# KirillKryukov/naf

Measured on AMD Instinct MI355X. Metric: unnaf GB/s (uncompressed bases out) on 100 GB synthetic FASTA, higher is better.
Workload: dtype u8; 1 GPU; unnaf decode of a 100.0 GB synthetic-ACGT FASTA archive on one GPU (the size BASELINE.json's metric is quoted on; configs[1] at 10 GB rides along as cfg10_*), 100 records, 80-col lines; archive made in-run by the GPU ennaf; .naf 24739662224 B -> FASTA 99999995684 B, text + archive + decoded text resident in HBM; parallelism=one archive, one GPU, no data-path collective

## Files before the change

### naf_amd/csrc/emit.hip

```cpp
#include "ctx.h"
#include "wgscan.h"
#include "emit_core.h"
#include "packed.h"
#include <thread>

__device__ __forceinline__ void st_text16(u8 *p, const uint4 &v, int nt)
{
    if (nt) {
        u32x4 nv; nv.x = v.x; nv.y = v.y; nv.z = v.z; nv.w = v.w;
        __builtin_nontemporal_store(nv, (u32x4 *)p);
    } else *(uint4 *)p = v;
}

__global__ void k_len_flags(const u32 *units, u64 n, u64 *flag)
{
    u64 i = (u64)blockIdx.x * blockDim.x + threadIdx.x;
    if (i < n) flag[i] = units[i] != 0xFFFFFFFFu;
}
__global__ void k_len_acc(const u32 *units, u64 n, const u64 *ridx, u64 *rec_len, u64 N)
{
    u64 i = (u64)blockIdx.x * blockDim.x + threadIdx.x;
    if (i < n && ridx[i] < N) atomicAdd((unsigned long long *)&rec_len[ridx[i]], (unsigned long long)units[i]);
}

#define ZT_BYTES 16
#define ZT_TILE (256 * ZT_BYTES)
__device__ __forceinline__ u32 zero_byte_mask16(const u8 *p, u64 base, u64 n)
{
    u32 m = 0;
    if (base + ZT_BYTES <= n) {
        u64 a = ld64(p + base), b = ld64(p + base + 8);
#pragma unroll
        for (int i = 0; i < 8; i++) { if (((a >> (8 * i)) & 0xFF) == 0) m |= 1u << i; if (((b >> (8 * i)) & 0xFF) == 0) m |= 1u << (8 + i); }
    } else {
        for (int i = 0; i < ZT_BYTES; i++) if (base + i < n && p[base + i] == 0) m |= 1u << i;
    }
    return m;
}
__global__ __launch_bounds__(256) void k_zero_count(const u8 *p, u64 n, u64 *tile_cnt)
{
    __shared__ u64 lds[4];
    u64 base = (u64)blockIdx.x * ZT_TILE + (u64)threadIdx.x * ZT_BYTES;
    u64 c = base < n ? __popc(zero_byte_mask16(p, base, n)) : 0, tot;
    wg_scan_inclusive<u64, OpAdd>(c, &tot, lds);
    if (threadIdx.x == 0) tile_cnt[blockIdx.x] = tot;
}
__global__ __launch_bounds__(256) void k_zero_scatter(const u8 *p, u64 n, const u64 *tile_pre, u64 *pos_out, u64 cap)
{
    __shared__ u64 lds[4];
    u64 base = (u64)blockIdx.x * ZT_TILE + (u64)threadIdx.x * ZT_BYTES;
    u32 m = base < n ? zero_byte_mask16(p, base, n) : 0;
    u64 c = __popc(m), tot;
    u64 incl = wg_scan_inclusive<u64, OpAdd>(c, &tot, lds);
    u64 k = tile_pre[blockIdx.x] + incl - c;
    while (m) { int b = __ffs(m) - 1; m &= m - 1; if (k < cap) pos_out[k] = base + b; k++; }
}

#define MT_TILE (256 * 16)
__device__ __forceinline__ void mask_units16(const u8 *units, u64 base, u64 n, u32 w[4], u32 &sum, u32 &cnt)
{
    sum = 0; cnt = 0; w[0] = w[1] = w[2] = w[3] = 0xFFFFFFFFu;
    if (base >= n) return;
    const u64 a = ld64(units + base), b = ld64(units + base + 8);
    w[0] = (u32)a; w[1] = (u32)(a >> 32); w[2] = (u32)b; w[3] = (u32)(b >> 32);
    const u32 valid = n - base >= 16 ? 16u : (u32)(n - base);
#pragma unroll
    for (u32 k = 0; k < 4; k++) {
        if (valid < 4 * k + 4) { const u32 keep = valid > 4 * k ? valid - 4 * k : 0; w[k] |= keep ? 0xFFFFFFFFu << (8 * keep) : 0xFFFFFFFFu; }
        const u32 y = ~w[k];
        const u32 z = ~(((y & 0x7F7F7F7Fu) + 0x7F7F7F7Fu) | y | 0x7F7F7F7Fu);
        cnt += 4 - (u32)__popc(z);
        sum += __builtin_amdgcn_sad_u8(w[k], 0u, 0u) - 255u * (u32)__popc(z);
    }
}
__global__ __launch_bounds__(256) void k_mask_count(const u8 *units, u64 n, u64 *tile_sum, u64 *tile_cnt)
{
    __shared__ u64 lds[4];
    u64 base = (u64)blockIdx.x * MT_TILE + (u64)threadIdx.x * 16;
    u32 w[4], s32, c32; mask_units16(units, base, n, w, s32, c32);
    const u32 valid = base >= n ? 0u : (n - base >= 16 ? 16u : (u32)(n - base));
    u64 s = (u64)s32 + 255ull * (valid - c32), c = c32;
    u64 t1, t2;
    wg_scan_inclusive<u64, OpAdd>(s, &t1, lds);
    wg_scan_inclusive<u64, OpAdd>(c, &t2, lds);
    if (threadIdx.x == 0) { tile_sum[blockIdx.x] = t1; tile_cnt[blockIdx.x] = t2; }
}
__global__ __launch_bounds__(256) void k_mask_scatter(const u8 *units, u64 n, const u64 *tile_sum_pre, const u64 *tile_cnt_pre, u64 *toggles, u64 n_toggles)
{
    __shared__ u64 lds[4];
    if ((blockIdx.x + 1 < gridDim.x ? tile_cnt_pre[blockIdx.x + 1] : n_toggles) == tile_cnt_pre[blockIdx.x]) return;
    u64 base = (u64)blockIdx.x * MT_TILE + (u64)threadIdx.x * 16;
    u32 w[4], s32, c32; mask_units16(units, base, n, w, s32, c32);
    const u32 valid = base >= n ? 0u : (n - base >= 16 ? 16u : (u32)(n - base));
    u64 s = (u64)s32 + 255ull * (valid - c32), c = c32;
    u64 t;
    u64 si = wg_scan_inclusive<u64, OpAdd>(s, &t, lds);
    u64 ci = wg_scan_inclusive<u64, OpAdd>(c, &t, lds);
    if (!c32) return;
    u64 pos = tile_sum_pre[blockIdx.x] + si - s, k = tile_cnt_pre[blockIdx.x] + ci - c;
    for (u32 i = 0; i < valid; i++) { u32 u = (w[i >> 2] >> (8 * (i & 3))) & 0xFF; pos += u; if (u != 255) toggles[k++] = pos; }
}

#define MASK_RLE_SRC (48u * 1024u)
#define MASK_RLE_TOG 8192u
__global__ __launch_bounds__(256) void k_mask_rle_frame(const u8 *src, u32 len, u32 hdr, u64 expect_units, u64 *toggles, u32 cap, u64 *res)
{
    __builtin_amdgcn_s_setprio(3);
    extern __shared__ __attribute__((aligned(16))) u8 mbuf[];
    __shared__ u64 lds[4]; __shared__ u32 s_first;
    const u32 t = threadIdx.x;
    for (u32 i = t; i < len; i += 256) mbuf[i] = src[i];
    if (t == 0) s_first = 0xFFFFFFFFu;
    __syncthreads();
    const u32 nA = len > hdr ? (len - hdr) / 4 : 0;
    for (u32 i = t; i < nA; i += 256) {
        const u32 p = hdr + 4 * i, h = (u32)mbuf[p] | ((u32)mbuf[p + 1] << 8) | ((u32)mbuf[p + 2] << 16);
        if (!(((h >> 1) & 3) == 1 && !(h & 1) && mbuf[p + 3] == 255)) { atomicMin(&s_first, i); break; }
    }
    __syncthreads();
    const u32 F = s_first < nA ? s_first : nA;
    u64 mine = 0;
    for (u32 i = t; i < F; i += 256) { const u32 p = hdr + 4 * i; mine += ((u32)mbuf[p] | ((u32)mbuf[p + 1] << 8) | ((u32)mbuf[p + 2] << 16)) >> 3; }
    u64 units = 0;
    wg_scan_inclusive<u64, OpAdd>(mine, &units, lds);
    u64 base = 255ull * units;
    u32 pos = hdr + 4 * F, nt = 0; bool ok = true, done = false;
    while (ok && !done) {
        if (pos + 3 > len) { ok = false; break; }
        const u32 h = (u32)mbuf[pos] | ((u32)mbuf[pos + 1] << 8) | ((u32)mbuf[pos + 2] << 16);
        const u32 last = h & 1, type = (h >> 1) & 3, size = h >> 3;
        if (type == 1) {
            if (pos + 4 > len) { ok = false; break; }
            const u32 v = mbuf[pos + 3];
            if (v != 255) {
                if ((u64)nt + size > cap) { ok = false; break; }
                for (u32 k = t; k < size; k += 256) toggles[nt + k] = base + (u64)v * (k + 1);
                nt += size;
            }
            base += (u64)v * size; units += size; pos += 4;
        } else if (type == 0) {
            if ((u64)pos + 3 + size > len) { ok = false; break; }
            const u8 *rb = mbuf + pos + 3;
            const u32 per = (size + 255) / 256, lo = t * per < size ? t * per : size, hi = lo + per < size ? lo + per : size;
            u64 sm = 0, cn = 0;
            for (u32 k = lo; k < hi; k++) { const u32 u = rb[k]; sm += u; cn += u != 255; }
            u64 tot_s, tot_c;
            const u64 is = wg_scan_inclusive<u64, OpAdd>(sm, &tot_s, lds);
            const u64 ic = wg_scan_inclusive<u64, OpAdd>(cn, &tot_c, lds);
            if (nt + tot_c > cap) { ok = false; break; }
            u64 at = base + is - sm; u32 idx = nt + (u32)(ic - cn);
            for (u32 k = lo; k < hi; k++) { const u32 u = rb[k]; at += u; if (u != 255) toggles[idx++] = at; }
            base += tot_s; nt += (u32)tot_c; units += size; pos += 3 + size;
        } else ok = false;
        if (last) done = true;
    }
    ok = ok && done && pos == len && units == expect_units;
    if (t == 0) { res[0] = ok ? 1 : 0; res[1] = nt; res[2] = units; }
}

__device__ __forceinline__ void rec_size_of(u64 r, u64 len, const u64 *idz, const u64 *nmz, int has_ids, int has_names, int mode, u64 L, u32 *hdr, u64 *out)
{
    u64 h = 0;
    if (mode == EM_FASTA || mode == EM_FASTQ) {
        u64 idl = 0, nml = 0;
        if (has_ids) idl = idz[r] - (r ? idz[r - 1] + 1 : 0);
        if (has_names) nml = nmz[r] - (r ? nmz[r - 1] + 1 : 0);
        u64 name = has_ids ? idl + ((has_names && nml) ? 1 + nml : 0) : nml;
        h = 1 + name + 1;
    }
    u64 body;
    if (mode == EM_FASTQ) body = 2 * len + 4;
    else if (mode == EM_SEQUENCES) body = len + 1;
    else body = len ? len + (L ? (len + L - 1) / L : 1) : 0;
    *hdr = (u32)h; *out = h + body;
}
__global__ void k_rec_sizes(u64 N, const u64 *rec_len, const u64 *idz, const u64 *nmz, int has_ids, int has_names,
                            int mode, u64 L, u32 *hdr_len, u64 *out_size, u64 *base_size)
{
    u64 r = (u64)blockIdx.x * blockDim.x + threadIdx.x;
    if (r >= N) return;
    u64 len = rec_len[r];
    rec_size_of(r, len, idz, nmz, has_ids, has_names, mode, L, &hdr_len[r], &out_size[r]);
    base_size[r] = len;
}

#define SIDE_FUSED_N 4096u
struct SideJob { const u32 *res; u32 n_jobs; u32 cap[3], len[3];
                 const u8 *ids, *names; const u32 *lens; u64 ids_n, names_n, n_len;
                 u64 N, L; int has_ids, has_names, mode;
                 u64 *idz, *nmz, *rec_len, *rec_out, *rec_base, *status; u32 *hdr_len; };
__device__ u64 wg_zero_positions(const u8 *p, u64 n, u64 *pos, u64 cap, u64 *lds)
{
    u64 run = 0;
    for (u64 tb = 0; tb < n; tb += ZT_TILE) {
        const u64 base = tb + (u64)threadIdx.x * ZT_BYTES;
        u32 m = base < n ? zero_byte_mask16(p, base, n) : 0;
        u64 c = __popc(m), tot;
        const u64 incl = wg_scan_inclusive<u64, OpAdd>(c, &tot, lds);
        u64 k = run + incl - c;
        while (m) { int b = __ffs(m) - 1; m &= m - 1; if (k < cap) pos[k] = base + b; k++; }
        run += tot;
    }
    return run;
}
__global__ __launch_bounds__(256) void k_side_tables(SideJob J)
{
    __shared__ u64 lds[4];
    __shared__ unsigned long long s_len[SIDE_FUSED_N];
    const u32 t = threadIdx.x;
    bool ok = true;
    for (u32 q = 0; q < J.n_jobs; q++) ok = ok && J.res[4 * q] == 0 && J.res[4 * q + 1] == J.cap[q] && J.res[4 * q + 2] == J.len[q];
    if (!ok) { if (t == 0) J.status[0] = 0; return; }
    for (u32 r = t; r < SIDE_FUSED_N; r += 256) s_len[r] = 0;
    const u64 n_ids = J.has_ids ? wg_zero_positions(J.ids, J.ids_n, J.idz, J.N, lds) : 0;
    const u64 n_names = J.has_names ? wg_zero_positions(J.names, J.names_n, J.nmz, J.N, lds) : 0;
    u64 nrec = 0;
    for (u64 b = 0; b < J.n_len; b += 256) {
        const u64 i = b + t; const u32 u = i < J.n_len ? J.lens[i] : 0xFFFFFFFFu;
        u64 f = i < J.n_len && u != 0xFFFFFFFFu, tot;
        const u64 incl = wg_scan_inclusive<u64, OpAdd>(f, &tot, lds);
        const u64 ridx = nrec + incl - f;
        if (i < J.n_len && ridx < J.N) atomicAdd(&s_len[ridx], (unsigned long long)u);
        nrec += tot;
    }
    __syncthreads();
    u64 run_out = 0, run_base = 0;
    for (u64 b = 0; b < J.N; b += 256) {
        const u64 r = b + t; u64 len = 0, o = 0, tot_o, tot_b; u32 hd = 0;
        if (r < J.N) { len = s_len[r]; rec_size_of(r, len, J.idz, J.nmz, J.has_ids, J.has_names, J.mode, J.L, &hd, &o); }
        const u64 io = wg_scan_inclusive<u64, OpAdd>(o, &tot_o, lds), ib = wg_scan_inclusive<u64, OpAdd>(len, &tot_b, lds);
        if (r < J.N) { J.rec_len[r] = len; J.hdr_len[r] = hd; J.rec_out[r] = run_out + io - o; J.rec_base[r] = run_base + ib - len; }
        run_out += tot_o; run_base += tot_b;
    }
    if (t == 0) {
        J.rec_len[J.N] = 0; J.rec_out[J.N] = run_out; J.rec_base[J.N] = run_base;
// ... 432 lines not shown
    }
    const u32 Lp1_32 = (P.L + 1) >> 32 ? 0 : (u32)(P.L + 1);
    auto geo_lds = [&](u64 r, u64 &ro, u64 &rn, u64 &len, u64 &base, u64 &ho, u32 &hl) {
        u32 i = (u32)(r - rlo); ro = s_ro[i]; rn = s_ro[i + 1]; len = s_len[i]; base = s_base[i]; hl = s_hl[i]; ho = s_ho[i];
    };
    GeoGlobal geo_g(P);
    for (u64 tile = span_first; tile <= span_last; tile += 4096) {
        u64 p0 = tile + (u64)threadIdx.x * 16;
        if (p0 > span_last) continue;
        u32 nbytes = P.out_end - p0 < 16 ? (u32)(P.out_end - p0) : 16;
        u8 *o = out + (p0 - P.out_begin);
        if (in_lds) {
            u32 lo_ = 0, hi_ = (u32)nrec; while (lo_ < hi_) { u32 mid = (lo_ + hi_) >> 1; if (s_ro[mid] <= p0) lo_ = mid + 1; else hi_ = mid; }
            compose_chunk<FOURBIT>(P, geo_lds, p0, nbytes, rlo + lo_ - 1, klo, khi, any_toggle, Lp1_32, o);
        } else {
            u64 r = upper_bound_u64(P.rec_out, rlo, rhi + 1, p0) - 1;
            compose_chunk<FOURBIT>(P, geo_g, p0, nbytes, r, klo, khi, any_toggle, Lp1_32, o);
        }
    }
}

#define ER_STAGE 24576u
template <bool FOURBIT, u32 ER_LANES, u32 WGT>
__global__ __launch_bounds__(WGT) void k_emit_fastq_records(EmitP P, u8 *out)
{
    constexpr u32 ER_READS = WGT / ER_LANES, STAGE = ER_STAGE / (256u / WGT);
    __shared__ __attribute__((aligned(16))) u8 stage[STAGE + 32];
    const u32 g = threadIdx.x & (ER_LANES - 1);
    const u64 r0 = (u64)blockIdx.x * ER_READS, r = r0 + threadIdx.x / ER_LANES;
    const u64 rend = r0 + ER_READS < P.N ? r0 + ER_READS : P.N;
    const u64 wbase = P.rec_out[r0], wspan = P.rec_out[rend] - wbase;
    const bool in_lds = wspan <= STAGE;
    if (r < P.N) {
        const u64 len = P.rec_len[r], base = P.rec_base[r];
        const u32 hl = P.hdr_len[r];
        u8 *o = in_lds ? stage + (P.rec_out[r] - wbase) : out + P.rec_out[r];
        u64 ids0 = 0, idl = 0, nm0 = 0, nml = 0;
        if (P.has_ids) { ids0 = r ? P.idz[r - 1] + 1 : 0; idl = P.idz[r] - ids0; }
        if (P.has_names) { nm0 = r ? P.nmz[r - 1] + 1 : 0; nml = P.nmz[r] - nm0; }
        if (g == 0) { o[0] = P.hdr_char; o[hl - 1] = '\n'; }
        if (P.has_ids) {
            group_copy<ER_LANES>(o + 1, P.ids + ids0, idl, g);
            if (P.has_names && nml) { if (g == 0) o[1 + idl] = P.sep; group_copy<ER_LANES>(o + 2 + idl, P.names + nm0, nml, g); }
        } else group_copy<ER_LANES>(o + 1, P.names + nm0, nml, g);
        u8 *os = o + hl;
        for (u64 i = (u64)g * 16; i < len; i += 16 * ER_LANES) {
            u64 lo, hi; bases16<FOURBIT>(P, base + i, lo, hi);
            store_upto16(os + i, lo, hi, len - i < 16 ? (u32)(len - i) : 16u);
        }
        if (g == 0) { os[len] = '\n'; os[len + 1] = '+'; os[len + 2] = '\n'; os[2 * len + 3] = '\n'; }
        group_copy<ER_LANES>(os + len + 3, P.qual + base, len, g);
    }
    if (!in_lds) return;
    __syncthreads();
    u8 *dst = out + wbase; const u32 n = (u32)wspan;
    u32 head = (u32)((16 - ((uintptr_t)dst & 15)) & 15); if (head > n) head = n;
    if (threadIdx.x < head) dst[threadIdx.x] = stage[threadIdx.x];
    u32 words = (n - head) >> 4;
    for (u32 w = threadIdx.x; w < words; w += WGT) {
        u64 a, b2; __builtin_memcpy(&a, stage + head + 16 * w, 8); __builtin_memcpy(&b2, stage + head + 16 * w + 8, 8);
        uint4 v; v.x = (u32)a; v.y = (u32)(a >> 32); v.z = (u32)b2; v.w = (u32)(b2 >> 32);
        st_text16(dst + head + 16 * w, v, P.nt_store);
    }
    for (u32 k = head + 16 * words + threadIdx.x; k < n; k += WGT) dst[k] = stage[k];
}

#define EMIT_TOG_LDS 256u
struct TileIdx { u64 gline, k, khi; u32 col, fast; };
#define TI_HDR 0xFFFFFFFFu
struct TileFlat { u64 q0, A, q1, A1, q2, qf; };
struct TileFlatE { u64 base, a1_addr; u32 a1_sh, K0, K1, d1, d2, qoff, par0, pad; };
static_assert(sizeof(TileFlatE) == sizeof(TileFlat), "the derived record replaces the raw one in place");
#define FLAT_QM 4096
#define TILE_WG 255
__global__ __launch_bounds__(256) void k_tile_index(EmitP P, u64 ntiles, TileIdx *ti, u64 *tr, u32 *list, u32 *count, TileFlat *tsig, u32 spare, u32 *list2)
{
    __shared__ u64 s_k[256], s_r[256];
    const u64 t = (u64)blockIdx.x * TILE_WG + threadIdx.x;
    const u64 p = P.out_begin + t * 4096;
    TileIdx x; x.fast = 0; x.gline = 0; x.khi = 0; x.k = P.n_toggles; x.col = TI_HDR;
    TileFlat f; f.q0 = f.A = f.q1 = f.A1 = f.q2 = f.qf = 0;
    u64 r = ~0ull; u32 cbits = 1;
    const bool inside = t < ntiles && p < P.out_end;
    if (inside) {
        u64 g;
        if (P.mode == EM_SEQ) { r = 0; x.col = 0; g = p; x.gline = p; }
        else {
            r = upper_bound_u64(P.rec_out, 0, P.N + 1, p) - 1;
            u64 off = p - P.rec_out[r], hl = P.hdr_len[r], len = P.rec_len[r], j = 0;
            if (off >= hl) {
                u64 q = off - hl;
                if (P.mode == EM_FASTA && P.L) {
                    u64 line = q / (P.L + 1), col = q - line * (P.L + 1);
                    j = line * P.L + (col < P.L ? col : P.L);
                    if (P.L < 0xFFFFFFF0ull) { x.gline = P.rec_base[r] + line * P.L; x.col = (u32)col; }
                } else if (P.mode != EM_FASTQ) { j = q; x.col = 0; x.gline = P.rec_base[r] + q; }
                if (j > len) j = len;
            }
            g = P.rec_base[r] + j;
        }
        x.k = P.masking ? upper_bound_u64(P.toggles, 0, P.n_toggles, g) : 0;
        if (tsig) {
            const FlatStream *si = (const FlatStream *)P.fsi;
            const u64 q = g >> 1;
            u64 lo, hi, gs = q >> 13; if (gs >= P.fslots) gs = P.fslots - 1;
            if (si[gs].q0 <= q) { lo = gs; hi = gs + 1; u64 st = 1; while (hi < P.fslots && si[hi].q0 <= q) { lo = hi; st <<= 1; hi = lo + st; } if (hi > P.fslots) hi = P.fslots; }
            else { hi = gs; u64 st = 1; lo = gs - 1; while (lo > 0 && si[lo].q0 > q) { hi = lo; st <<= 1; lo = lo > st ? lo - st : 0; } }
            while (hi - lo > 1) { const u64 mid = (lo + hi) >> 1; if (si[mid].q0 <= q) lo = mid; else hi = mid; }
            f.q0 = si[lo].q0; f.A = si[lo].A; f.qf = q;
            if (P.fcls) {
                u32 c = 3; u64 b = lo >> 2; const u64 nb = P.fslots >> 2, qe = q + 2048 + 16;
                for (u32 k = 0; k < 6 && b < nb && si[4 * b].q0 <= qe; k++, b++) c &= P.fcls[b];
                if (b < nb && si[4 * b].q0 <= qe) c = 0;
                cbits = c;
            }
            u64 cs = lo + 1;
            while (cs < P.fslots && si[cs + 1].q0 == si[cs].q0) cs++;
            f.q1 = si[cs].q0; f.A1 = cs < P.fslots ? si[cs].A : 0;
            u64 ce = cs < P.fslots ? cs + 1 : cs;
            while (ce < P.fslots && si[ce + 1].q0 == si[ce].q0) ce++;
            f.q2 = si[ce].q0;
        }
    }
    s_k[threadIdx.x] = x.k; s_r[threadIdx.x] = r;
    __syncthreads();
    if (threadIdx.x == TILE_WG) return;
    TileFlatE e; e.base = (u64)P.fsrc; e.a1_addr = (u64)P.fsrc; e.a1_sh = 4; e.K0 = e.K1 = 0; e.d1 = e.d2 = 0x7FFFFFFFu; e.qoff = 0; e.par0 = 0; e.pad = 0;
    if (t >= ntiles) {
        if (t == ntiles) { tr[t] = ~0ull; ti[t] = x; if (tsig && spare) *(TileFlatE *)&tsig[t] = e; }
        else if (tsig && t < ntiles + spare) { ti[t].fast = 0; *(TileFlatE *)&tsig[t] = e; }
        return;
    }
    tr[t] = r;
    if (!inside) { ti[t] = x; if (tsig) *(TileFlatE *)&tsig[t] = e; list[atomicAdd(count, 1u)] = (u32)t; return; }
    const u64 r_next = s_r[threadIdx.x + 1];
    x.khi = s_k[threadIdx.x + 1];
    const bool wrap = P.mode == EM_FASTA && P.L != 0;
    bool fast = x.col != TI_HDR && r == r_next && P.out_begin + (t + 1) * 4096 <= P.out_end && !P.force_slow && (!wrap || P.L >= 16);
    bool packed = false;
    if (tsig) {
        packed = fast && (cbits & 2);
        if (fast && !(cbits & 1)) fast = false;
        if (fast) {
            fast = f.qf + 2048 + 16 < f.q2 || f.q2 == f.q1;
            if (P.ftail && f.qf + 2048 + 16 >= P.ftail_q) fast = false;
            if (f.q2 != f.q1 && (f.A1 > f.A ? f.A1 - f.A : f.A - f.A1) >= (1ull << 29)) fast = false;
        }
        if (fast) {
            const u64 gline = x.gline;
            const u64 dd1 = f.q1 - f.qf, dd2 = f.q2 - f.qf;
            e.d1 = dd1 > 0x7FFFFFFFull ? 0x7FFFFFFFu : (u32)dd1; e.d2 = dd2 > 0x7FFFFFFFull ? 0x7FFFFFFFu : (u32)dd2;
            const u64 T0 = f.A - 4 * (f.qf - f.q0), T1 = f.A1 + 4 * (u64)e.d1;
            const bool two = f.q2 != f.q1;
            const u64 tmin = two && T1 < T0 ? T1 : T0;
            const u64 ub = (tmin - 40 - 4 * (u64)FLAT_QM) & ~7ull;
            e.base = (u64)P.fsrc + (u64)((i64)ub >> 3);
            e.K0 = (u32)(T0 - 40 - ub); e.K1 = two ? (u32)(T1 - 40 - ub) : e.K0;
            e.qoff = (u32)((gline >> 1) - f.qf); e.par0 = (u32)gline & 1u;
            const u64 t1 = (f.A1 < 40 ? 40 : f.A1) - 40;
            e.a1_addr = (u64)P.fsrc + (t1 >> 3); e.a1_sh = (u32)(t1 & 7) + 4;
        }
        *(TileFlatE *)&tsig[t] = e;
    }
    x.fast = fast ? 1u : (packed ? 2u : 0u);
    ti[t] = x;
    if (!fast) { if (packed) list2[atomicAdd(count + 1, 1u)] = (u32)t; else list[atomicAdd(count, 1u)] = (u32)t; }
}

template <bool FOURBIT>
__device__ __forceinline__ void emit_tile_body(const EmitP &P, const TileIdx &a, u8 *out_tile)
{
    __shared__ u64 s_tog[EMIT_TOG_LDS];
    const u32 ntog = (u32)(a.khi - a.k < EMIT_TOG_LDS ? a.khi - a.k : EMIT_TOG_LDS);
    const bool use_tog = P.masking && a.k < a.khi && a.khi - a.k <= EMIT_TOG_LDS;
    if (use_tog) { for (u32 i = threadIdx.x; i < ntog; i += 256) s_tog[i] = P.toggles[a.k + i]; __syncthreads(); }
    const u32 lane16 = threadIdx.x * 16;
    u64 g0; u32 nl_b = 64;
    if (P.mode == EM_FASTA && P.L != 0) {
        const u32 Lp1 = (u32)P.L + 1;
        u32 c = a.col + lane16, dl;
        if (Lp1 < 32768) dl = __umulhi(c, P.Ldiv_magic); else dl = c >= Lp1 ? 1u : 0u;
        u32 col = c - dl * Lp1;
// ... 614 lines not shown
}

struct SideCall {
    const u8 *d_naf; UnnafPlan &pl; const naf_gpu_header &h; EmitP &P;
    bool want_names = false;
    int sec[3] = { S_IDS, S_NAMES, S_LEN }; bool wanted[3] = { false, false, true };
    u8 *pre[3] = { nullptr, nullptr, nullptr };
    u64 *rec_len = nullptr;
    u64 tot[2] = { 0, 0 };
    bool mask_meanwhile = false, mask_ran = false; int rc_mask = 0; char mask_err[sizeof(naf_gpu_ctx::err)];
};

struct SectionJobs { const u8 *src[3]; size_t len[3], cap[3]; u8 *dst[3]; int k[3]; int m; };
static int section_jobs(naf_gpu_ctx *x, const SideCall &S, SectionJobs &j)
{
    const naf_gpu_header &h = S.h;
    j.m = 0;
    for (int k = 0; k < 3; k++) {
        const int s = S.sec[k];
        if (!S.wanted[k] || h.orig_size[s] == 0) continue;
        u8 *b = (u8 *)arena_alloc(x, h.orig_size[s] + 32); if (!b) return NAF_GPU_ENOMEM;
        j.src[j.m] = S.d_naf + h.payload_off[s]; j.len[j.m] = h.comp_size[s]; j.dst[j.m] = b; j.cap[j.m] = h.orig_size[s]; j.k[j.m++] = k;
    }
    return 0;
}

static int side_small_batch(naf_gpu_ctx *x, SideCall &S)
{
    SectionJobs j; bool ok[3];
    int r = section_jobs(x, S, j); if (r) return r;
    if (!j.m) return 0;
    if ((r = zstd_small_batch(x, j.m, j.src, j.len, j.dst, j.cap, ok))) return r;
    for (int q = 0; q < j.m; q++) if (ok[q]) S.pre[j.k[q]] = j.dst[q];
    return 0;
}

static int side_ids_names(naf_gpu_ctx *x, SideCall &S, int which)
{
    const naf_gpu_header &h = S.h; EmitP &P = S.P;
    const u64 N = h.n_sequences;
    int r;
    if ((which & 1) && S.wanted[0]) {
        u8 *b = S.pre[0]; u64 *z = nullptr;
        if (h.orig_size[S_IDS] == 0) return ctx_fail(x, NAF_GPU_EFORMAT, "corrupted ids - not 0-terminated\n");
        if (!b && (r = load_section(x, S.d_naf, h, S_IDS, h.orig_size[S_IDS], "ids", &b, S.pl.frame_head[S_IDS]))) return r;
        if ((r = zero_positions(x, b, h.orig_size[S_IDS], N, &z, false))) return r;
        P.ids = b; P.idz = z;
    }
    if ((which & 2) && S.wanted[1]) {
        u8 *b = S.pre[1]; u64 *z = nullptr;
        if (h.orig_size[S_NAMES] == 0) return ctx_fail(x, NAF_GPU_EFORMAT, "corrupted names - not 0-terminated\n");
        if (!b && (r = load_section(x, S.d_naf, h, S_NAMES, h.orig_size[S_NAMES], "names", &b, S.pl.frame_head[S_NAMES]))) return r;
        if ((r = zero_positions(x, b, h.orig_size[S_NAMES], N, &z, true))) return r;
        P.names = b; P.nmz = z;
    }
    return 0;
}

static int side_lengths(naf_gpu_ctx *x, SideCall &S)
{
    const naf_gpu_header &h = S.h;
    const u64 N = h.n_sequences;
    int r;
    u8 *lens = S.pre[2];
    if (!lens && (r = load_section(x, S.d_naf, h, S_LEN, h.orig_size[S_LEN], "lengths", &lens, S.pl.frame_head[S_LEN]))) return r;
    u64 n_len = h.orig_size[S_LEN] / 4;
    u64 *flag = arena_new<u64>(x, n_len + 2), *rec_len = S.rec_len = arena_new<u64>(x, N + 1);
    if (!flag || !rec_len) return NAF_GPU_ENOMEM;
    HIP_TRY(x, hipMemsetAsync(rec_len, 0, (N + 1) * 8, x->stream));
    if (n_len) LAUNCH(x, "unnaf_len_flags", k_len_flags, cdiv(n_len, 256), 256, 0, (const u32 *)lens, n_len, flag);
    if ((r = scan_exclusive_u64(x, flag, n_len, flag + n_len + 1))) return r;
    if (n_len) LAUNCH(x, "unnaf_len_acc", k_len_acc, cdiv(n_len, 256), 256, 0, (const u32 *)lens, n_len, (const u64 *)flag, rec_len, N);
    u64 nrec = 0;
    if ((r = ctx_readback(x, &nrec, flag + n_len + 1, 8))) return r;
    if (nrec < N) return ctx_fail(x, NAF_GPU_EFORMAT, "corrupted lengths: %llu records described, %llu expected", (unsigned long long)nrec, (unsigned long long)N);
    return 0;
}

static int mask_rle_frame(naf_gpu_ctx *x, SideCall &S, bool *done)
{
    const naf_gpu_header &h = S.h; EmitP &P = S.P;
    const u64 cs = h.comp_size[S_MASK], n_mask = h.orig_size[S_MASK];
    *done = false;
    if (!(cs >= 4 && cs <= MASK_RLE_SRC && n_mask >= 2 * cs) || ctx_opt_is(x, "MASK_RLE", '0')) return 0;
    const u8 fhd = S.pl.frame_head[S_MASK][0];
    const u32 fcs_flag = fhd >> 6, single = (fhd >> 5) & 1;
    const u32 hdr_size = 1 + (single ? 0 : 1) + (fcs_flag == 0 ? single : (fcs_flag == 1 ? 2 : (fcs_flag == 2 ? 4 : 8)));
    if ((fhd & 0x0F) || hdr_size >= cs) return 0;
    u64 *tg = arena_new<u64>(x, MASK_RLE_TOG + 1), *d_res = arena_new<u64>(x, 4);
    if (!tg || !d_res) return NAF_GPU_ENOMEM;
    LAUNCH(x, "unnaf_mask_rle", k_mask_rle_frame, 1, 256, (u32)((cs + 15) & ~15ull), S.d_naf + h.payload_off[S_MASK], (u32)cs, hdr_size, n_mask, tg, MASK_RLE_TOG, d_res);
    u64 res[3] = { 0, 0, 0 };
    int r = ctx_readback(x, res, d_res, 24); if (r) return r;
    if (res[0] == 1) { P.toggles = tg; P.n_toggles = res[1]; *done = true; }
    return 0;
}

static int mask_toggles(naf_gpu_ctx *x, SideCall &S)
{
    const naf_gpu_header &h = S.h; EmitP &P = S.P;
    int r; bool done;
    u8 *mu = nullptr; const u64 n_mask = h.orig_size[S_MASK];
    if ((r = mask_rle_frame(x, S, &done)) || done) return r;
    if ((r = load_section(x, S.d_naf, h, S_MASK, n_mask, "mask", &mu, S.pl.frame_head[S_MASK]))) return r;
    u64 tiles = (n_mask + MT_TILE - 1) / MT_TILE;
    u64 *ts = arena_new<u64>(x, tiles + 2), *tc = arena_new<u64>(x, tiles + 2);
    if (!ts || !tc) return NAF_GPU_ENOMEM;
    if (tiles) LAUNCH(x, "unnaf_mask_count", k_mask_count, tiles, 256, 0, (const u8 *)mu, n_mask, ts, tc);
    if ((r = scan_exclusive_u64(x, ts, tiles, (u64 *)nullptr))) return r;
    if ((r = scan_exclusive_u64(x, tc, tiles, tc + tiles + 1))) return r;
    u64 ntog = 0;
    if ((r = ctx_readback(x, &ntog, tc + tiles + 1, 8))) return r;
    u64 *tg = arena_new<u64>(x, ntog + 1);
    if (!tg) return NAF_GPU_ENOMEM;
    if (tiles) LAUNCH(x, "unnaf_mask_scatter", k_mask_scatter, tiles, 256, 0, (const u8 *)mu, n_mask, (const u64 *)ts, (const u64 *)tc, tg, ntog);
    P.toggles = tg; P.n_toggles = ntog;
    return 0;
}

static void side_mask_meanwhile(naf_gpu_ctx *c, SideCall &S)
{
    if (!S.mask_meanwhile) return;
    S.mask_ran = true; S.rc_mask = mask_toggles(c, S);
    if (S.rc_mask) memcpy(S.mask_err, c->err, sizeof c->err);
}

static int side_fused_launch(naf_gpu_ctx *x, SideCall &S, u64 st[6], bool *done)
{
    const naf_gpu_header &h = S.h; EmitP &P = S.P;
    const u64 N = h.n_sequences;
    SectionJobs j; u8 *buf[3] = { nullptr, nullptr, nullptr };
    int r = section_jobs(x, S, j); if (r) return r;
    SideJob J; memset(&J, 0, sizeof J);
    for (int q = 0; q < j.m; q++) { J.cap[q] = (u32)j.cap[q]; J.len[q] = (u32)j.len[q]; buf[j.k[q]] = j.dst[q]; }
    u32 *d_res = nullptr;
    if ((r = zstd_small_launch(x, j.m, j.src, j.len, j.dst, j.cap, &d_res))) return r;
    J.res = d_res; J.n_jobs = (u32)j.m;
    J.ids = buf[0]; J.ids_n = h.orig_size[S_IDS]; J.names = buf[1]; J.names_n = h.orig_size[S_NAMES];
    J.lens = (const u32 *)buf[2]; J.n_len = h.orig_size[S_LEN] / 4;
    J.N = N; J.L = P.L; J.has_ids = P.has_ids; J.has_names = P.has_names; J.mode = P.mode;
    J.idz = P.has_ids ? arena_new<u64>(x, N + 1) : nullptr; J.nmz = P.has_names ? arena_new<u64>(x, N + 1) : nullptr;
    J.rec_len = arena_new<u64>(x, N + 1); J.hdr_len = arena_new<u32>(x, N + 1);
    J.rec_out = arena_new<u64>(x, N + 2); J.rec_base = arena_new<u64>(x, N + 2); J.status = arena_new<u64>(x, 8);
    if ((P.has_ids && !J.idz) || (P.has_names && !J.nmz) || !J.rec_len || !J.hdr_len || !J.rec_out || !J.rec_base || !J.status) return NAF_GPU_ENOMEM;
    LAUNCH(x, "unnaf_side_tables", k_side_tables, 1, 256, 0, J);
    if ((r = ctx_readback(x, st, J.status, 6 * sizeof(u64)))) return r;
    if (st[0] != 1) return 0;
    P.ids = buf[0]; P.idz = J.idz; P.names = buf[1]; P.nmz = J.nmz;
    P.rec_len = J.rec_len; P.hdr_len = J.hdr_len; P.rec_out = J.rec_out; P.rec_base = J.rec_base;
    *done = true;
    return 0;
}

static int side_fused_tables(naf_gpu_ctx *c, SideCall &S, naf_gpu_ctx *aux, bool *done)
{
    const naf_gpu_header &h = S.h; EmitP &P = S.P;
    const u64 N = h.n_sequences;
    *done = false;
    bool fits = !ctx_opt_is(c, "SIDE_FUSED", '0') && N <= SIDE_FUSED_N && h.orig_size[S_LEN] % 4 == 0;
    for (int k = 0; k < 3; k++) if (S.wanted[k] && (!zstd_small_fits(h.comp_size[S.sec[k]], h.orig_size[S.sec[k]]) || h.orig_size[S.sec[k]] == 0)) fits = false;
    if (!fits) return 0;
    u64 st[6] = { 0, 0, 0, 0, 0, 0 };
    int rf = 0;
    if (aux) {
        CtxJoinGuard joined{ aux };
        ctx_worker_start(aux, [&] { rf = side_fused_launch(aux, S, st, done); });
        side_mask_meanwhile(c, S);
        ctx_worker_join(aux);
        if (rf) ctx_take_error(c, aux);
    } else rf = side_fused_launch(c, S, st, done);
    if (rf || !*done) return rf;
    if (st[3] < N) return ctx_fail(c, NAF_GPU_EFORMAT, "corrupted lengths: %llu records described, %llu expected", (unsigned long long)st[3], (unsigned long long)N);
    if (P.has_ids && st[1] < N) return ctx_fail(c, NAF_GPU_EFORMAT, "currupted ids - can't read id %llu\n", (unsigned long long)st[1]);
    if (P.has_names && st[2] < N) return ctx_fail(c, NAF_GPU_EFORMAT, "corrupted names - can't read name %llu\n", (unsigned long long)st[2]);
// ... 547 lines not shown
```

Before: 4269 GB/s.

## Stream mask RLE frame from global memory and reuse per-block record lookup

The single-workgroup mask RLE decoder no longer copies the whole compressed frame into dynamic LDS. It scans runs of all-255 RLE blocks straight from global memory in register batches and stages raw blocks through a fixed 16 KB LDS buffer. This lifts the 48 KB size limit, so larger mask frames take the fast path, with a cap on non-run blocks. Separately, k_tile_index does one record binary search per block and reuses that record's fields for tiles in the same record, adding extra loads per thread when tiles cross record boundaries.

```diff
diff --git a/naf_amd/csrc/emit.hip b/naf_amd/csrc/emit.hip
--- a/naf_amd/csrc/emit.hip
+++ b/naf_amd/csrc/emit.hip
@@ -101,37 +101,48 @@
     for (u32 i = 0; i < valid; i++) { u32 u = (w[i >> 2] >> (8 * (i & 3))) & 0xFF; pos += u; if (u != 255) toggles[k++] = pos; }
 }
 
-#define MASK_RLE_SRC (48u * 1024u)
 #define MASK_RLE_TOG 8192u
+#define MASK_RLE_RUN 8u
+#define MASK_RLE_STAGE (16u * 1024u)
+#define MASK_RLE_OTHER 2048u
 __global__ __launch_bounds__(256) void k_mask_rle_frame(const u8 *src, u32 len, u32 hdr, u64 expect_units, u64 *toggles, u32 cap, u64 *res)
 {
     __builtin_amdgcn_s_setprio(3);
-    extern __shared__ __attribute__((aligned(16))) u8 mbuf[];
-    __shared__ u64 lds[4]; __shared__ u32 s_first;
+    __shared__ __attribute__((aligned(16))) u8 stage[MASK_RLE_STAGE];
+    __shared__ u64 lds[4]; __shared__ u32 s_first[2];
     const u32 t = threadIdx.x;
-    for (u32 i = t; i < len; i += 256) mbuf[i] = src[i];
-    if (t == 0) s_first = 0xFFFFFFFFu;
-    __syncthreads();
-    const u32 nA = len > hdr ? (len - hdr) / 4 : 0;
-    for (u32 i = t; i < nA; i += 256) {
-        const u32 p = hdr + 4 * i, h = (u32)mbuf[p] | ((u32)mbuf[p + 1] << 8) | ((u32)mbuf[p + 2] << 16);
-        if (!(((h >> 1) & 3) == 1 && !(h & 1) && mbuf[p + 3] == 255)) { atomicMin(&s_first, i); break; }
-    }
-    __syncthreads();
-    const u32 F = s_first < nA ? s_first : nA;
-    u64 mine = 0;
-    for (u32 i = t; i < F; i += 256) { const u32 p = hdr + 4 * i; mine += ((u32)mbuf[p] | ((u32)mbuf[p + 1] << 8) | ((u32)mbuf[p + 2] << 16)) >> 3; }
-    u64 units = 0;
-    wg_scan_inclusive<u64, OpAdd>(mine, &units, lds);
-    u64 base = 255ull * units;
-    u32 pos = hdr + 4 * F, nt = 0; bool ok = true, done = false;
+    const u64 g = (u64)src;
+    u32 pos = hdr, nt = 0, other = 0, round = 0; u64 units = 0, base = 0; bool ok = true, done = false;
     while (ok && !done) {
-        if (pos + 3 > len) { ok = false; break; }
-        const u32 h = (u32)mbuf[pos] | ((u32)mbuf[pos + 1] << 8) | ((u32)mbuf[pos + 2] << 16);
+        u64 mine = 0;
+        for (;;) {
+            const u32 left = (len - pos) / 4, n = left < 256 * MASK_RLE_RUN ? left : 256 * MASK_RLE_RUN;
+            u32 *first = &s_first[round++ & 1];
+            if (t == 0) *first = n;
+            __syncthreads();
+            u32 h[MASK_RLE_RUN], bad = n;
+#pragma unroll
+            for (u32 j = 0; j < MASK_RLE_RUN; j++) { const u32 i = j * 256 + t; h[j] = i < n ? ldg_at_unaligned<u32>(g + pos + 4 * i) : 0u; }
+#pragma unroll
+            for (u32 j = MASK_RLE_RUN; j-- > 0; ) { const u32 i = j * 256 + t; if (i < n && (h[j] & 0xFF000007u) != 0xFF000002u) bad = i; }
+            if (bad < n) atomicMin(first, bad);
+            __syncthreads();
+            const u32 F = *first;
+#pragma unroll
+            for (u32 j = 0; j < MASK_RLE_RUN; j++) if (j * 256 + t < F) mine += (h[j] & 0xFFFFFFu) >> 3;
+            pos += 4 * F;
+            if (F < 256 * MASK_RLE_RUN) break;
+        }
+        u64 run = 0;
+        wg_scan_inclusive<u64, OpAdd>(mine, &run, lds);
+        units += run; base += 255ull * run;
+        if (len - pos < 3 || other == MASK_RLE_OTHER) { ok = false; break; }
+        other++;
+        const u32 h = (u32)src[pos] | ((u32)src[pos + 1] << 8) | ((u32)src[pos + 2] << 16);
         const u32 last = h & 1, type = (h >> 1) & 3, size = h >> 3;
         if (type == 1) {
-            if (pos + 4 > len) { ok = false; break; }
-            const u32 v = mbuf[pos + 3];
+            if (len - pos < 4) { ok = false; break; }
+            const u32 v = src[pos + 3];
             if (v != 255) {
                 if ((u64)nt + size > cap) { ok = false; break; }
                 for (u32 k = t; k < size; k += 256) toggles[nt + k] = base + (u64)v * (k + 1);
@@ -139,18 +150,28 @@
             }
             base += (u64)v * size; units += size; pos += 4;
         } else if (type == 0) {
-            if ((u64)pos + 3 + size > len) { ok = false; break; }
-            const u8 *rb = mbuf + pos + 3;
-            const u32 per = (size + 255) / 256, lo = t * per < size ? t * per : size, hi = lo + per < size ? lo + per : size;
-            u64 sm = 0, cn = 0;
-            for (u32 k = lo; k < hi; k++) { const u32 u = rb[k]; sm += u; cn += u != 255; }
-            u64 tot_s, tot_c;
-            const u64 is = wg_scan_inclusive<u64, OpAdd>(sm, &tot_s, lds);
-            const u64 ic = wg_scan_inclusive<u64, OpAdd>(cn, &tot_c, lds);
-            if (nt + tot_c > cap) { ok = false; break; }
-            u64 at = base + is - sm; u32 idx = nt + (u32)(ic - cn);
-            for (u32 k = lo; k < hi; k++) { const u32 u = rb[k]; at += u; if (u != 255) toggles[idx++] = at; }
-            base += tot_s; nt += (u32)tot_c; units += size; pos += 3 + size;
+            if (len - pos - 3 < size) { ok = false; break; }
+            const u32 rb = pos + 3;
+            for (u32 o = 0; o < size && ok; o += MASK_RLE_STAGE) {
+                const u32 n = size - o < MASK_RLE_STAGE ? size - o : MASK_RLE_STAGE;
+                __syncthreads();
+                for (u32 i = 8 * t; i < n; i += 8 * 256) {
+                    if (i + 8 <= n) *(u64 *)(stage + i) = ldg_at_unaligned<u64>(g + rb + o + i);
+                    else for (u32 k = i; k < n; k++) stage[k] = src[rb + o + k];
+                }
+                __syncthreads();
+                const u32 per = (n + 255) / 256, lo = t * per < n ? t * per : n, hi = lo + per < n ? lo + per : n;
+                u64 sm = 0, cn = 0;
+                for (u32 k = lo; k < hi; k++) { const u32 u = stage[k]; sm += u; cn += u != 255; }
+                u64 tot_s, tot_c;
+                const u64 is = wg_scan_inclusive<u64, OpAdd>(sm, &tot_s, lds);
+                const u64 ic = wg_scan_inclusive<u64, OpAdd>(cn, &tot_c, lds);
+                if (nt + tot_c > cap) { ok = false; break; }
+                u64 at = base + is - sm; u32 idx = nt + (u32)(ic - cn);
+                for (u32 k = lo; k < hi; k++) { const u32 u = stage[k]; at += u; if (u != 255) toggles[idx++] = at; }
+                base += tot_s; nt += (u32)tot_c;
+            }
+            units += size; pos += 3 + size;
         } else ok = false;
         if (last) done = true;
     }
@@ -749,22 +770,30 @@
     TileFlat f; f.q0 = f.A = f.q1 = f.A1 = f.q2 = f.qf = 0;
     u64 r = ~0ull; u32 cbits = 1;
     const bool inside = t < ntiles && p < P.out_end;
+    u64 r0 = 0, r0_out = 0, r0_next = 0, r0_hl = 0, r0_len = 0, r0_base = 0;
+    if (P.mode != EM_SEQ && P.N) {
+        r0 = upper_bound_u64(P.rec_out, 0, P.N + 1, P.out_begin + (u64)blockIdx.x * TILE_WG * 4096) - 1;
+        if (r0 >= P.N) r0 = P.N - 1;
+        r0_out = P.rec_out[r0]; r0_next = P.rec_out[r0 + 1]; r0_hl = P.hdr_len[r0]; r0_len = P.rec_len[r0]; r0_base = P.rec_base[r0];
+    }
     if (inside) {
         u64 g;
         if (P.mode == EM_SEQ) { r = 0; x.col = 0; g = p; x.gline = p; }
         else {
-            r = upper_bound_u64(P.rec_out, 0, P.N + 1, p) - 1;
-            u64 off = p - P.rec_out[r], hl = P.hdr_len[r], len = P.rec_len[r], j = 0;
+            const bool same = p < r0_next;
+            r = same ? r0 : upper_bound_u64(P.rec_out, r0 + 1, P.N + 1, p) - 1;
+            const u64 rbase = same ? r0_base : P.rec_base[r];
+            u64 off = p - (same ? r0_out : P.rec_out[r]), hl = same ? r0_hl : P.hdr_len[r], len = same ? r0_len : P.rec_len[r], j = 0;
             if (off >= hl) {
                 u64 q = off - hl;
                 if (P.mode == EM_FASTA && P.L) {
                     u64 line = q / (P.L + 1), col = q - line * (P.L + 1);
                     j = line * P.L + (col < P.L ? col : P.L);
-                    if (P.L < 0xFFFFFFF0ull) { x.gline = P.rec_base[r] + line * P.L; x.col = (u32)col; }
-                } else if (P.mode != EM_FASTQ) { j = q; x.col = 0; x.gline = P.rec_base[r] + q; }
+                    if (P.L < 0xFFFFFFF0ull) { x.gline = rbase + line * P.L; x.col = (u32)col; }
+                } else if (P.mode != EM_FASTQ) { j = q; x.col = 0; x.gline = rbase + q; }
                 if (j > len) j = len;
             }
-            g = P.rec_base[r] + j;
+            g = rbase + j;
         }
         x.k = P.masking ? upper_bound_u64(P.toggles, 0, P.n_toggles, g) : 0;
         if (tsig) {
@@ -1545,14 +1574,14 @@
     const naf_gpu_header &h = S.h; EmitP &P = S.P;
     const u64 cs = h.comp_size[S_MASK], n_mask = h.orig_size[S_MASK];
     *done = false;
-    if (!(cs >= 4 && cs <= MASK_RLE_SRC && n_mask >= 2 * cs) || ctx_opt_is(x, "MASK_RLE", '0')) return 0;
+    if (!(cs >= 4 && cs <= 0x7FFFFFFFull && n_mask >= 2 * cs) || ctx_opt_is(x, "MASK_RLE", '0')) return 0;
     const u8 fhd = S.pl.frame_head[S_MASK][0];
     const u32 fcs_flag = fhd >> 6, single = (fhd >> 5) & 1;
     const u32 hdr_size = 1 + (single ? 0 : 1) + (fcs_flag == 0 ? single : (fcs_flag == 1 ? 2 : (fcs_flag == 2 ? 4 : 8)));
     if ((fhd & 0x0F) || hdr_size >= cs) return 0;
     u64 *tg = arena_new<u64>(x, MASK_RLE_TOG + 1), *d_res = arena_new<u64>(x, 4);
     if (!tg || !d_res) return NAF_GPU_ENOMEM;
-    LAUNCH(x, "unnaf_mask_rle", k_mask_rle_frame, 1, 256, (u32)((cs + 15) & ~15ull), S.d_naf + h.payload_off[S_MASK], (u32)cs, hdr_size, n_mask, tg, MASK_RLE_TOG, d_res);
+    LAUNCH(x, "unnaf_mask_rle", k_mask_rle_frame, 1, 256, 0, S.d_naf + h.payload_off[S_MASK], (u32)cs, hdr_size, n_mask, tg, MASK_RLE_TOG, d_res);
     u64 res[3] = { 0, 0, 0 };
     int r = ctx_readback(x, res, d_res, 24); if (r) return r;
     if (res[0] == 1) { P.toggles = tg; P.n_toggles = res[1]; *done = true; }
```

New measurement: 4404 GB/s, median of 6. 1.03x the previous value.
